# JiawangBian/SC-SfMLearner-Release

Measured on AMD Instinct MI355X. Metric: train images/sec (+ warp-loss ms/step) KITTI 256x832 RN18, higher is better.
Workload: dtype f32; 1 GPU; configs[1]: kitti 256x832, batch 12/GPU, 2 refs (seq 3), ResNet18 DispNet + ResNet18 PoseNet, ssim+mask+auto-mask, zeros padding, 1 scale; global_batch=12, parallelism=1 GPU, memory_format=contiguous (NCHW)

## Files before the change

### __graft_entry__.py

```python
import os
import sys

ROOT = os.path.dirname(os.path.abspath(__file__))
PKG = os.path.join(ROOT, "sc-sfmlearner-release_amd")
for p in (ROOT, PKG):
    if p not in sys.path:
        sys.path.insert(0, p)


REPORT_ORDER = ("dgrad", "vlog", "wrw", "decb", "enceval", "val", "dvis", "", "nets", "eval", "odom", "enc", "stem", "snip",
                "vis", "prep")


def build() -> None:
    from scsfm_hip import _lib, build as hip_build
    from scsfm_hip.libraries import ADDED, BEYOND, BY_NAME, FURTHER, LATER, NEWER, NEWEST, NEXT, REGISTRY
    libs = {row.name: _lib.CLib(hip_build.build_lib(row.name, force=False), row.header, row.abi, row.prefix)
            for row in REGISTRY}
    assert libs[""]._dll.scsfm_abi_version() == _lib.ABI_VERSION
    import inverse_warp
    import loss_functions
    import models
    from scsfm_hip import decoder, depth_eval, depth_vis, encoder, odometry, prepare, snippets, visualise
    from scsfm_hip import conv_wrw, decoder_bias, decoder_dgrad, encoder_eval, validation, validation_log
    from scsfm_hip import conv1x1, encoder_frozen, fusion, meshing, optim, raycast, tracking, training_state
    from scsfm_hip import confidence, rolling, similarity
    from oracle import scsfm_oracle
    for row in ADDED + FURTHER:
        print(f"[{row.tag}] {libs[row.name].path}: ABI {row.abi}, {len(libs[row.name].decls)} symbols of "
              f"include/{os.path.basename(row.header)}")
    for row in NEWER + NEWEST:
        print(f"[{row.tag}] {libs[row.name].path}: {len(libs[row.name].decls)} entry points resolved (ABI {row.abi})")
    for row in LATER:
        print(f"[{row.tag}] {libs[row.name].path}: {len(libs[row.name].decls)} entry points resolved")
    for row in NEXT:
        print(f"[{row.tag}] {libs[row.name].path}: {len(libs[row.name].decls)} entry points resolved (ABI {row.abi})")
    for name in REPORT_ORDER:
        print(f"[{BY_NAME[name].tag}] {libs[name].path}: {len(libs[name].decls)} entry points resolved")
        if name == "dgrad":
            for row in BEYOND:
                print(f"[{row.tag}] {libs[row.name].path}: {len(libs[row.name].decls)} entry points resolved (ABI "
                      f"{row.abi})")


def smoke() -> None:
    import torch

    import loss_functions as LF
    from oracle import scsfm_oracle as O
    from scsfm_hip import _lib, synth

    assert torch.cuda.is_available(), "smoke() needs a HIP device"
    lib = _lib.get()
    assert lib.path.endswith("libscsfm_hip.so")
    dev = torch.device("cuda:0")
    d = synth.make_batch(2, 128, 416, n_ref=2, seed=0, depth="smooth")

    def leaves(device):
        mv = lambda t: t.to(device).clone().requires_grad_(True)
        return ([mv(t) for t in d["tgt_depth"]], [[mv(t) for t in r] for r in d["ref_depths"]],
                [mv(p) for p in d["poses"]], [mv(p) for p in d["poses_inv"]])

    td, rd, ps, pi = leaves(dev)
    tgt, refs, K = d["tgt_img"].to(dev), [r.to(dev) for r in d["ref_imgs"]], d["intrinsics"].to(dev)
    photo, geom = LF.compute_photo_and_geometry_loss(tgt, refs, K, td, rd, ps, pi, 1, 1, 1, 1, "zeros")
    smooth = LF.compute_smooth_loss(td, tgt, rd, refs)
    (photo + 0.1 * smooth + 0.5 * geom).backward()
    torch.cuda.synchronize()

    td_c, rd_c, ps_c, pi_c = leaves("cpu")
    photo_c, geom_c = O.photo_and_geometry_loss(d["tgt_img"], d["ref_imgs"], d["intrinsics"], td_c, rd_c, ps_c, pi_c,
                                                1, 1, 1, 1, "zeros")
    smooth_c = O.smooth_loss(td_c, d["tgt_img"], rd_c, d["ref_imgs"])
    (photo_c + 0.1 * smooth_c + 0.5 * geom_c).backward()
    for name, a, b in (("photo", photo, photo_c), ("geom", geom, geom_c), ("smooth", smooth, smooth_c)):
        err = abs(float(a) - float(b))
        print(f"[smoke] {name}: hip {float(a):.7f} oracle {float(b):.7f} |d| {err:.2e}")
        assert err <= 1e-5, name
    pairs = [("g_tgt_depth", td[0].grad, td_c[0].grad), ("g_ref0_depth", rd[0][0].grad, rd_c[0][0].grad),
             ("g_ref1_depth", rd[1][0].grad, rd_c[1][0].grad), ("g_pose0", ps[0].grad, ps_c[0].grad),
             ("g_pose_inv1", pi[1].grad, pi_c[1].grad)]
    for name, a, b in pairs:
        scale = float(b.abs().max())
        bad = ((a.cpu() - b).abs() > 0.01 * scale).double().mean().item()
        print(f"[smoke] {name}: scale {scale:.3e} share of entries off by >1% of scale {bad:.2e}")
        assert bad <= 2e-3, name
    import torch.nn as nn
    from scsfm_hip import encoder as E
    assert _lib.get_stem().path.endswith("libscsfm_stem.so")
    xs = torch.randn(2, 4, 6, 8, device=dev)
    bn_a, bn_b = nn.BatchNorm2d(4).to(dev).train(), nn.BatchNorm2d(4).to(dev).train()
    f0, pooled = E.bn_act(xs, bn_a, pool=True)
    f0_ref = E.bn_act(xs, bn_b)
    assert torch.equal(f0, f0_ref) and torch.equal(pooled, E.max_pool(f0_ref))
    print("[smoke] stem: fused BatchNorm / ReLU / max-pool equals the separate ops")
    import numpy as np
    from scsfm_hip import visualise as V
    assert _lib.get_vis().path.endswith("libscsfm_vis.so")
    ramp = torch.linspace(0.05, 12.0, 70).reshape(2, 5, 7)
    for cmap, max_value in (("bone", None), ("rainbow", 10)):
        got = V.colourise(ramp.to(dev), colormap=cmap, max_value=max_value).cpu().numpy()
        table = V.colour_table(cmap)
        r = ramp.numpy()
        d = r.reshape(2, -1).max(axis=1)[:, None, None] if max_value is None else np.float32(max_value)
        xa = (r / d).astype(np.float32) * np.float32(len(table))
        want = table[np.clip(xa.astype(np.int64), 0, len(table) - 1)]
        assert got.shape == (2, 5, 7, 4) and np.array_equal(got, want), cmap
    print("[smoke] vis: bone and rainbow pictures of a ramp equal the table lookup")
    from scsfm_hip import depth_vis as DV
# ... 10 lines not shown
    print("[smoke] dvis: the magma picture of a depth ramp equals the table lookup")
    from scsfm_hip import validation as VA
    assert _lib.get_val().path.endswith("libscsfm_val.so")
    f32 = np.float32
    rng = np.random.default_rng(0)
    gt_v = rng.uniform(0.05, 90.0, (2, 20, 60)).astype(f32)
    disp_v = rng.uniform(0.01, 1.5, (2, 10, 30)).astype(f32)
    res = VA.depth_errors(torch.from_numpy(gt_v).to(dev), torch.from_numpy(disp_v).to(dev), "kitti", is_disp=True)
    got = VA.batch_mean(res)
    y1, y2, x1, x2 = int(0.40810811 * 20), int(0.99189189 * 20), int(0.03594771 * 60), int(0.96405229 * 60)
    want = np.zeros(6)
    for g, dsp in zip(gt_v, disp_v):
        p = (f32(1) / dsp)[np.arange(20) // 2][:, np.arange(60) // 2]
        ok = np.zeros((20, 60), bool)
        ok[y1:y2, x1:x2] = True
        ok &= (g > f32(0.1)) & (g < f32(80))
        g, p = g[ok], np.clip(p[ok], f32(1e-3), f32(80))
        p = p * np.sort(g)[(g.size - 1) // 2] / np.sort(p)[(p.size - 1) // 2]
        t = np.maximum(g / p, p / g)
        e = np.abs(g - p).astype(np.float64)
        want += [e.mean(), (e / g).mean(), (e * e / g).mean(), (t < 1.25).mean(), (t < 1.25 ** 2).mean(),
                 (t < 1.25 ** 3).mean()]
    want /= 2
    print(f"[smoke] val: abs_rel hip {got[1]:.7f} numpy {want[1]:.7f}; a1 hip {got[3]:.7f} numpy {want[3]:.7f}")
    assert res.count.cpu().numpy().min() > 100 and np.allclose(got, want, rtol=1e-6, atol=0), (got, want)
    table = VA.ValidationTable(4, dev)
    rows_v = [(0.25, 0.002, 1.5), (0.5, float("nan"), 0.75), (0.125, 0.004, 0.25)]
    for i, vals_v in zip((0, 1, 3), rows_v):
        table.add_losses(i, *torch.tensor(vals_v, device=dev))
    mean_v, n_v = table.finish()
    sums_v = [0.0] * 4
    for p_v, s_v, g_v in rows_v:
        sums_v = [a + float(f32(b)) for a, b in zip(sums_v, (p_v, p_v, s_v, g_v))]
    want_v = [s / 3 for s in sums_v] + [0.0] * 3
    print(f"[smoke] val: table of 3 present rows of 4: photo {mean_v[1]:.7f} host {want_v[1]:.7f}, smooth {mean_v[2]} "
          f"(a NaN row), geometry {mean_v[3]:.7f} host {want_v[3]:.7f}")
    assert n_v == 3 and np.isnan(mean_v[2]) and mean_v[:2] + mean_v[3:] == want_v[:2] + want_v[3:], (mean_v, want_v)
    import torch.nn.functional as F
    from scsfm_hip import encoder_eval as EE
    assert _lib.get_enceval().path.endswith("libscsfm_enceval.so")
    bn_e = nn.BatchNorm2d(4).to(dev)
    with torch.no_grad():
        bn_e.running_mean.copy_(torch.tensor([0.5, -1.0, 0.0, 2.0]))
        bn_e.running_var.copy_(torch.tensor([0.25, 1.0, 4.0, 0.5]))
        bn_e.weight.copy_(torch.tensor([1.0, -0.5, 2.0, 0.0]))
        bn_e.bias.copy_(torch.tensor([0.0, 0.1, -0.2, 0.3]))
    bn_e.eval()
    with torch.no_grad():
        f0_e, pooled_e = EE.bn_act(xs, bn_e, pool=True)
        want_e = F.relu(bn_e(xs))
        assert torch.equal(f0_e, EE.bn_act(xs, bn_e)) and torch.equal(pooled_e, F.max_pool2d(f0_e, 3, 2, 1))
        assert torch.equal(pooled_e, EE.max_pool(f0_e))
    err_e = float((f0_e - want_e).abs().max())
    print(f"[smoke] enceval: eval-mode BatchNorm / ReLU / max-pool, max |fused - ATen| {err_e:.2e}")
    assert err_e <= 1e-5
    from scsfm_hip import decoder_bias as DB
    assert _lib.get_decb().path.endswith("libscsfm_decb.so")
    conv_b = nn.Conv2d(4, 3, 3).to(dev)
    xb = torch.randn(2, 4, 9, 11, device=dev)
    want_b = F.pad(F.elu(conv_b(xb)), (1, 1, 1, 1), mode="reflect")
    want_h = 10 * torch.sigmoid(conv_b(xb)) + 0.01
    (want_b.sum() + want_h.sum()).backward()
    want_gb = conv_b.bias.grad.clone()
    conv_b.bias.grad = None
    raw = F.conv2d(xb, conv_b.weight, None)
    got_b, got_h = DB.elu_pad(raw, conv_b.bias), DB.disp_head(raw, conv_b.bias, 10, 0.01)
    (got_b.sum() + got_h.sum()).backward()
    err_b = float((conv_b.bias.grad - want_gb).abs().max() / want_gb.abs().max())
    print(f"[smoke] decb: bias folded into elu_pad and disp_head, relative bias-gradient difference {err_b:.2e}")
    assert torch.equal(got_b, want_b) and float((got_h - want_h).abs().max()) <= 1e-6 and err_b <= 1e-5
    _smoke_wrw(dev)
    _smoke_vlog(dev)
    _smoke_dgrad(dev)
    _smoke_fbn(dev)
    _smoke_opt(dev)
    _smoke_pw(dev)
    _smoke_fuse(dev)
    _smoke_mesh(dev)
    _smoke_cast(dev)
    _smoke_track(dev)
    _smoke_conf(dev)
    _smoke_roll(dev)
    _smoke_sim3(dev)
    print("[smoke] ok")


def _smoke_cast(dev) -> None:
    import numpy as np
    import torch

    from scsfm_hip import _lib
    from scsfm_hip import fusion as FU
    assert _lib.get_cast().path.endswith("libscsfm_cast.so")
    nx, ny, nz = 12, 10, 9
    z, y, x = np.meshgrid(np.arange(nz), np.arange(ny), np.arange(nx), indexing="ij")
    t = ((np.sqrt((x - 5.3) ** 2 + (y - 4.6) ** 2 + (z - 4.1) ** 2) - 3.2) / 3).clip(-1, 1).astype(np.float32)
    vol = FU.Volume((nx, ny, nz), (-0.6, -0.5, 0.3), 0.1, device=dev)
    vol.planes[0].copy_(torch.from_numpy(t))
    vol.planes[1].fill_(1.0)
    vol.planes[2:].fill_(0.5)
    centre = np.array([-0.6 + 0.1 * 5.8, -0.5 + 0.1 * 5.1, 0.3 + 0.1 * 4.6])
    c2w = np.concatenate([np.eye(3), [[centre[0]], [centre[1]], [-0.3]]], axis=1)[None]
    K = torch.tensor([[20.0, 0, 8.0], [0, 20.0, 6.0], [0, 0, 1]], device=dev)
    args = (torch.from_numpy(c2w).to(dev), K, (12, 16), 0.0, 1.5)
    got, plain = vol.raycast(*args), vol.raycast(*args, cull=False)
    for a, b in zip(got, plain):
        assert torch.equal(a.view(torch.uint8), b.view(torch.uint8))
    hits = int((got.depth > 0).sum())
    d = float(got.depth[0, 6, 8])
    want = centre[2] + 0.3 - 0.32
    assert hits > 40 and abs(d - want) < 0.025, (hits, d, want)
    assert float(got.normal[0, 2, 6, 8]) < -0.99 and int(got.shade[0, 6, 8]) >= 250 and got.rgb[0, 6, 8].tolist() == [128] * 3
    print(f"[smoke] cast: a sphere in a 12 x 10 x 9 volume from a 12 x 16 camera: {hits} pixels with a hit, the same bits "
          f"with and without the brick cull; the central depth {d:.4f} against {want:.4f}")


def _smoke_conf(dev) -> None:
    import numpy as np
    import torch

    from scsfm_hip import _lib, confidence
    from scsfm_hip import fusion as FU
    assert _lib.get_conf().path.endswith("libscsfm_conf.so")
    K = torch.tensor([[16.0, 0, 7.5], [0, 16.0, 5.5], [0, 0, 1]], device=dev)
    c2w = np.stack([np.concatenate([np.eye(3), [[0.125 * k], [0.0], [0.0]]], axis=1) for k in range(3)])
    c2w = torch.from_numpy(c2w).to(dev)
    depth = torch.full((3, 12, 16), 2.0, device=dev)
    flat = confidence.weights(depth, c2w, K, radius=1, is_disp=False, max_depth=4.0)
    met = int((flat == 1).sum())
    assert bool(((flat == 0) | (flat == 1)).all()) and met > 3 * 10 * 13, met
    depth[1, 4:8, 6:10] = 1.5
    w = confidence.weights(depth, c2w, K, radius=1, is_disp=False, max_depth=4.0)
    low = float(w[1, 4:8, 6:10].max())
    assert low < 0.9 and torch.equal(w[1, 9:11], flat[1, 9:11]), low
    vols = []
    for weight in (None, torch.ones_like(w), w):
        vol = FU.Volume((24, 16, 12), (-1.0, -0.8, 1.6), 0.1, device=dev)
        vol.integrate(depth, None, c2w, K, is_disp=False, max_depth=4.0, weight=weight)
        vols.append(vol.planes)
    assert torch.equal(vols[0].view(torch.int32), vols[1].view(torch.int32)) and not torch.equal(vols[0], vols[2])
    assert float(vols[2][1].max()) <= 3.0 and float(vols[2][1].max()) > 1.0
    print(f"[smoke] conf: three flat 12 x 16 frames a pixel apart: {met} weights of exactly 1, the rest 0; a nearer patch "
          f"weighs at most {low:.4f}; a weight of ones fuses to the unweighted bits")


def _smoke_roll(dev) -> None:
    import numpy as np
    import torch

    from scsfm_hip import _lib, rolling
    assert _lib.get_roll().path.endswith("libscsfm_roll.so")
    K = torch.tensor([[16.0, 0, 7.5], [0, 16.0, 5.5], [0, 0, 1]], device=dev)
    c2w = np.stack([np.concatenate([np.eye(3), [[0.125 * k], [0.0], [0.0]]], axis=1) for k in range(3)])
    c2w = torch.from_numpy(c2w).to(dev)
    yy = torch.arange(12, device=dev, dtype=torch.float32)[None, :, None]
    depth = (1.0 + 0.05 * yy).expand(3, 12, 16).contiguous()
    vol = rolling.RollingVolume((24, 16, 20), (-1.0, -0.75, 0.5), 0.0625, device=dev)
    assert vol.nbytes == 40 * 24 * 16 * 20 and vol.offset == (0, 0, 0) and vol.origin == vol.origin0
    vol.integrate(depth, None, c2w, K, is_disp=False, max_depth=4.0)
    before = vol.planes.clone()
    full = vol.extract(1.0)[0]
    out = vol.shift((8, 0, 10), 1.0)[0]
    want = torch.zeros_like(before)
    want[:, :10, :, :16] = before[:, 10:, :, 8:]
    assert torch.equal(vol.planes.view(torch.int32), want.view(torch.int32))
    assert vol.offset == (8, 0, 10) and vol.origin == (-0.5, -0.75, 1.125)
# ... 91 lines not shown
    w[:, :, 10:] = 0
    vol = FU.Volume((nx, ny, nz), (-0.6, -0.5, 0.3), 0.1, device=dev)
    vol.planes[0].copy_(torch.from_numpy(t))
    vol.planes[1].copy_(torch.from_numpy(w))
    vol.planes[2:].fill_(0.5)
    seen, neg = w >= 1, t < 0
    corner = lambda a, k: a[(k >> 2):nz - 1 + (k >> 2), ((k >> 1) & 1):ny - 1 + ((k >> 1) & 1), (k & 1):nx - 1 + (k & 1)]
    n_vert, is_axial = 0, []
    edge = np.zeros((nz, ny, nx, 7), bool)
    for e, k in enumerate((1, 2, 4, 3, 5, 6, 7)):
        dz, dy, dx = k >> 2, (k >> 1) & 1, k & 1
        a = (slice(0, nz - dz), slice(0, ny - dy), slice(0, nx - dx))
        b = (slice(dz, nz), slice(dy, ny), slice(dx, nx))
        edge[a + (e,)] = seen[a] & seen[b] & (neg[a] != neg[b])
    n_vert = int(edge.sum())
    is_axial = (np.flatnonzero(edge.reshape(-1)) % 7) < 3
    n_tri = 0
    for tet in ((0, 1, 3, 7), (0, 1, 5, 7), (0, 2, 3, 7), (0, 2, 6, 7), (0, 4, 5, 7), (0, 4, 6, 7)):
        ok = np.logical_and.reduce([corner(seen, k) for k in tet])
        inside = sum(corner(neg, k).astype(int) for k in tet)
        n_tri += int((ok & ((inside == 1) | (inside == 3))).sum() + 2 * (ok & (inside == 2)).sum())
    xyz, rgb, tri = vol.extract_mesh(1.0)
    pts, cols = vol.extract(1.0)
    assert xyz.shape == (n_vert, 3) and rgb.shape == (n_vert, 3) and tri.shape == (n_tri, 3) and n_tri > 100
    assert tri.dtype == torch.int32 and int(tri.min()) >= 0 and int(tri.max()) < n_vert
    keep = torch.from_numpy(is_axial).to(dev)
    assert torch.equal(xyz[keep].view(torch.int32), pts.view(torch.int32)) and torch.equal(rgb[keep], cols)
    print(f"[smoke] mesh: a cut sphere in a 12 x 10 x 9 volume: {n_vert} vertices and {n_tri} triangles as numpy counts "
          f"them; the {len(pts)} vertices on the grid's edges equal the surface points bit for bit")


def _smoke_fuse(dev) -> None:
    import numpy as np
    import torch

    from scsfm_hip import _lib
    from scsfm_hip import fusion as FU
    assert _lib.get_fuse().path.endswith("libscsfm_fuse.so")
    f32 = np.float32
    rng = np.random.default_rng(11)
    H, W, dims, origin, voxel, trunc, max_depth = 6, 8, (12, 10, 9), (-0.6, -0.5, 0.3), f32(0.1), f32(0.3), f32(3.0)
    K = np.array([[6, 0, 3.5], [0, 6, 2.5], [0, 0, 1]], f32)
    c2w = np.array([[[1, 0, 0, x], [0, 1, 0, 0.05], [0, 0, 1, 0]] for x in (-0.25, 0.5)], np.float64)
    disp = (1 / (0.8 + 0.02 * rng.random((2, 1, H, W)))).astype(f32)
    disp[0, 0, 1, 2], disp[1, 0, 4, 5] = 0.01, np.nan
    img = rng.standard_normal((2, 3, H, W)).astype(f32)
    vol = FU.Volume(dims, origin, float(voxel), float(trunc), max_weight=64.0, device=dev, frames_per_launch=2)
    vol.integrate(*(torch.from_numpy(a).to(dev) for a in (disp, img, c2w, K)), is_disp=True, near=0.05,
                  max_depth=float(max_depth))
    axis = lambda o, n: f32(o) + (np.arange(n, dtype=f32) + f32(0.5)) * voxel
    x, y, z = axis(origin[0], 12)[None, None, :], axis(origin[1], 10)[None, :, None], axis(origin[2], 9)[:, None, None]
    planes = np.zeros((5, 9, 10, 12), f32)
    t, w = planes[0], planes[1]
    with np.errstate(all="ignore"):
        for f in range(2):
            tr = (-c2w[f, :, 3]).astype(f32)
            qx, qy, qz = ((x + f32(0) * y) + f32(0) * z) + tr[0], ((f32(0) * x + y) + f32(0) * z) + tr[1], \
                ((f32(0) * x + f32(0) * y) + z) + tr[2]
            a, b = ((K[0, 0] * qx) / qz + K[0, 2]) + f32(0.5), ((K[1, 1] * qy) / qz + K[1, 2]) + f32(0.5)
            ok = (qz > f32(0.05)) & (a >= 0) & (a < f32(W)) & (b >= 0) & (b < f32(H))
            px, py = np.where(ok, a, 0).astype(np.int32), np.where(ok, b, 0).astype(np.int32)
            d = f32(1) / disp[f, 0][py, px]
            sdf = d - qz
            ok &= (d > 0) & (d <= max_depth) & ~(sdf < -trunc)
            w1 = w + f32(1)
            t[...] = np.where(ok, (t * w + np.minimum(f32(1), sdf / trunc)) / w1, t)
            for ch in range(3):
                col = img[f, ch][py, px] * f32(0.225) + f32(0.45)
                planes[2 + ch] = np.where(ok, (planes[2 + ch] * w + col) / w1, planes[2 + ch])
            w[...] = np.where(ok, np.minimum(w1, f32(64)), w)
    assert planes.dtype == f32 and w.max() == 2 and torch.equal(vol.planes.cpu(), torch.from_numpy(planes))
    seen, neg = w >= 1, t < 0
    n_z = int((seen[:-1] & seen[1:] & (neg[:-1] != neg[1:])).sum())
    n_y = int((seen[:, :-1] & seen[:, 1:] & (neg[:, :-1] != neg[:, 1:])).sum())
    n_x = int((seen[:, :, :-1] & seen[:, :, 1:] & (neg[:, :, :-1] != neg[:, :, 1:])).sum())
    xyz, rgb = vol.extract(min_weight=1)
    assert xyz.shape == (n_x + n_y + n_z, 3) and rgb.shape == xyz.shape and n_z > 20
    zs = xyz[:, 2].cpu().numpy()
    print(f"[smoke] fuse: two frames into a 12 x 10 x 9 volume equal the numpy restatement bit for bit; {len(zs)} surface "
          f"points, depth {zs.min():.3f} .. {zs.max():.3f} of a surface at 0.80 .. 0.82")
    assert 0.75 < zs.min() and zs.max() < 0.87


def _smoke_pw(dev) -> None:
    import torch
    import torch.nn.functional as F

    from scsfm_hip import _lib
    from scsfm_hip import conv1x1 as PW
    assert _lib.get_pw().path.endswith("libscsfm_pw.so")
    g = torch.Generator().manual_seed(9)
    xp = torch.randn(2, 64, 7, 11, generator=g).to(dev).requires_grad_(True)
    wp = (torch.randn(128, 64, 1, 1, generator=g) / 8).to(dev).requires_grad_(True)
    gy = torch.randn(2, 128, 4, 6, generator=g).to(dev)
    old = torch.backends.cudnn.deterministic, torch.backends.cudnn.benchmark
    torch.backends.cudnn.deterministic, torch.backends.cudnn.benchmark = True, False
    try:
        y, y_ref = PW.conv1x1(xp, wp, None, 2), F.conv2d(xp, wp, None, 2)
    finally:
        torch.backends.cudnn.deterministic, torch.backends.cudnn.benchmark = old
    assert torch.equal(y, y_ref)
    gx_w, gw_w = PW.data_grad(gy, wp.detach(), 7, 11), PW.weight_grad(xp.detach(), gy, 2)
    gx_m, gw_m = torch.autograd.grad(y_ref, (xp, wp), gy)
    x64, w64 = (t.detach().double().requires_grad_(True) for t in (xp, wp))
    gx_64, gw_64 = torch.autograd.grad(F.conv2d(x64, w64, None, 2), (x64, w64), gy.double())
    xa, wa = (t.detach().double().abs().requires_grad_(True) for t in (xp, wp))
    sx_64, sw_64 = torch.autograd.grad(F.conv2d(xa, wa, None, 2), (xa, wa), gy.double().abs())
    u8 = 8 * 2.0 ** -24
    for name, got, miopen, want, s in (("weight", gw_w, gw_m, gw_64, sw_64), ("data", gx_w, gx_m, gx_64, sx_64)):
        err, err_m = (got - want).abs(), float((miopen - want).abs().max())
        print(f"[smoke] pw: {name} gradient of a 64 -> 128 stride-2 1x1 convolution, max |hip - fp64| "
              f"{float(err.max()):.2e} (MIOpen's {err_m:.2e})")
        assert bool((err <= 2 * err_m + u8 * s).all()), name
    assert bool((gx_w[:, :, 1::2, :] == 0).all()) and bool((gx_w[:, :, :, 1::2] == 0).all())
    if (64, 128, 2) in PW.ROUTED and (64, 128, 2) in PW.ROUTED_DGRAD:
        gx_f, gw_f = torch.autograd.grad(y, (xp, wp), gy)
        assert torch.equal(gx_f, gx_w) and torch.equal(gw_f, gw_w)


def _smoke_opt(dev) -> None:
    import numpy as np
    import torch

    from scsfm_hip import _lib
    from scsfm_hip import optim as OP
    assert _lib.get_opt().path.endswith("libscsfm_opt.so")
    f32 = np.float32
    g = torch.Generator().manual_seed(7)
    shapes, lrs, wd, betas, eps = ((7,), (4, 6), (2 * OP.CHUNK + 3,), (3, 5, 5)), (1e-3, 1e-2), 0.01, (0.9, 0.999), 1e-8
    host = [torch.randn(s, generator=g) for s in shapes]
    params = [torch.nn.Parameter(t.to(dev)) for t in host]
    opt = OP.Adam([{"params": params[:2], "lr": lrs[0]}, {"params": params[2:], "lr": lrs[1]}], betas=betas, eps=eps,
                  weight_decay=wd)
    p = [t.numpy().copy() for t in host]
    m, v = [np.zeros_like(a) for a in p], [np.zeros_like(a) for a in p]
    b1c, b2, b2c, e, w = f32(1.0 - betas[0]), f32(betas[1]), f32(1.0 - betas[1]), f32(eps), f32(wd)
    for step in (1, 2, 3):
        grads = [torch.randn(s, generator=g) for s in shapes]
        for q, gr in zip(params, grads):
            q.grad = gr.to(dev)
        opt.step()
        for k, gr in enumerate(grads):
            step_size = f32(lrs[k // 2] / (1 - betas[0] ** step))
            bc2_sqrt = f32((1 - betas[1] ** step) ** 0.5)
            gk = gr.numpy() + w * p[k]
            m[k] = m[k] + b1c * (gk - m[k])
            v[k] = v[k] * b2 + (b2c * gk) * gk
            p[k] = p[k] - step_size * (m[k] / (np.sqrt(v[k]) / bc2_sqrt + e))
    state = opt.state_dict()["state"]
    for k in range(4):
        assert p[k].dtype == f32 and torch.equal(params[k].detach().cpu(), torch.from_numpy(p[k])), k
        assert torch.equal(state[k]["exp_avg"].cpu(), torch.from_numpy(m[k])), k
        assert torch.equal(state[k]["exp_avg_sq"].cpu(), torch.from_numpy(v[k])), k
        assert float(state[k]["step"]) == 3.0
    print("[smoke] opt: three Adam steps of four tensors in one launch each equal the numpy restatement bit for bit")


def _smoke_fbn(dev) -> None:
    import torch
    import torch.nn as nn
    import torch.nn.functional as F

    from scsfm_hip import _lib
    from scsfm_hip import encoder_frozen as EF
    assert _lib.get_fbn().path.endswith("libscsfm_fbn.so")
    g = torch.Generator().manual_seed(5)
# ... 106 lines not shown
```

### sc-sfmlearner-release_amd/models/resnet_encoder.py

```python
from __future__ import absolute_import, division, print_function

import numpy as np
import torch
import torch.nn as nn


_encoder_ops = None


def _E():
    global _encoder_ops
    if _encoder_ops is None:
        from scsfm_hip import encoder
        _encoder_ops = encoder
    return _encoder_ops


_encoder_eval_ops = None


def _EV():
    global _encoder_eval_ops
    if _encoder_eval_ops is None:
        from scsfm_hip import encoder_eval
        _encoder_eval_ops = encoder_eval
    return _encoder_eval_ops


_encoder_frozen_ops = None


def _EF():
    global _encoder_frozen_ops
    if _encoder_frozen_ops is None:
        from scsfm_hip import encoder_frozen
        _encoder_frozen_ops = encoder_frozen
    return _encoder_frozen_ops


def _fused_applies(x, *bns):
    return x.is_cuda and _E().applies(x, *bns)


def _eval_applies(x, *bns):
    return x.is_cuda and _EV().applies(x, *bns)


def _frozen_applies(x, *bns, relu=True):
    return x.is_cuda and not any(bn.training for bn in bns) and _EF().applies(x, *bns, relu=relu)


def _bn_act(x, bn, act, identity=None):
    if _fused_applies(x, bn) and (identity is None or _fused_applies(identity)):
        return _E().bn_act(x, bn, identity, relu=act is not None)
    if _frozen_applies(x, bn, relu=act is not None) and (identity is None or _frozen_applies(identity)):
        return _EF().bn_act(x, bn, identity, relu=act is not None)
    if _eval_applies(x, bn) and (identity is None or _eval_applies(identity)):
        return _EV().bn_act(x, bn, identity, relu=act is not None)
    out = bn(x)
    if identity is not None:
        out = out + identity
    return out if act is None else act(out)


_conv1x1_ops = None


def _PW():
    global _conv1x1_ops
    if _conv1x1_ops is None:
        from scsfm_hip import conv1x1
        _conv1x1_ops = conv1x1
    return _conv1x1_ops


def _downsample(ds, x):
    conv, bn = ds[0], ds[1]
    hip = x.is_cuda and (bn.training or (_EF().is_frozen(bn) and _EF().enabled()))
    y = _PW().conv(conv, x) if hip else conv(x)
    return _bn_act(y, bn, None)


def _conv3x3(cin, cout, stride=1):
    return nn.Conv2d(cin, cout, kernel_size=3, stride=stride, padding=1, bias=False)


class BasicBlock(nn.Module):
    expansion = 1

    def __init__(self, inplanes, planes, stride=1, downsample=None):
        super().__init__()
        self.conv1 = _conv3x3(inplanes, planes, stride)
        self.bn1 = nn.BatchNorm2d(planes)
        self.relu = nn.ReLU(inplace=True)
        self.conv2 = _conv3x3(planes, planes)
        self.bn2 = nn.BatchNorm2d(planes)
        self.downsample = downsample

    def forward(self, x):
        identity = x if self.downsample is None else _downsample(self.downsample, x)
        out = _bn_act(self.conv1(x), self.bn1, self.relu)
        return _bn_act(self.conv2(out), self.bn2, self.relu, identity)

    def forward_reference(self, x):
        identity = x if self.downsample is None else self.downsample(x)
        out = self.relu(self.bn1(self.conv1(x)))
        out = self.bn2(self.conv2(out))
        return self.relu(out + identity)


class Bottleneck(nn.Module):
    expansion = 4

    def __init__(self, inplanes, planes, stride=1, downsample=None):
        super().__init__()
        self.conv1 = nn.Conv2d(inplanes, planes, kernel_size=1, bias=False)
        self.bn1 = nn.BatchNorm2d(planes)
        self.conv2 = _conv3x3(planes, planes, stride)
        self.bn2 = nn.BatchNorm2d(planes)
        self.conv3 = nn.Conv2d(planes, planes * 4, kernel_size=1, bias=False)
        self.bn3 = nn.BatchNorm2d(planes * 4)
        self.relu = nn.ReLU(inplace=True)
        self.downsample = downsample

    def forward(self, x):
        identity = x if self.downsample is None else _downsample(self.downsample, x)
        out = _bn_act(self.conv1(x), self.bn1, self.relu)
        out = _bn_act(self.conv2(out), self.bn2, self.relu)
        return _bn_act(self.conv3(out), self.bn3, self.relu, identity)

    def forward_reference(self, x):
        identity = x if self.downsample is None else self.downsample(x)
        out = self.relu(self.bn1(self.conv1(x)))
        out = self.relu(self.bn2(self.conv2(out)))
        out = self.bn3(self.conv3(out))
        return self.relu(out + identity)


class ResNet(nn.Module):

    def __init__(self, block, layers, num_classes=1000, num_input_images=1):
        super().__init__()
        self.inplanes = 64
        self.conv1 = nn.Conv2d(num_input_images * 3, 64, kernel_size=7, stride=2, padding=3, bias=False)
        self.bn1 = nn.BatchNorm2d(64)
        self.relu = nn.ReLU(inplace=True)
        self.maxpool = nn.MaxPool2d(kernel_size=3, stride=2, padding=1)
        self.layer1 = self._make_layer(block, 64, layers[0])
        self.layer2 = self._make_layer(block, 128, layers[1], stride=2)
        self.layer3 = self._make_layer(block, 256, layers[2], stride=2)
        self.layer4 = self._make_layer(block, 512, layers[3], stride=2)
        self.avgpool = nn.AdaptiveAvgPool2d((1, 1))
        self.fc = nn.Linear(512 * block.expansion, num_classes)
        for m in self.modules():
            if isinstance(m, nn.Conv2d):
                nn.init.kaiming_normal_(m.weight, mode='fan_out', nonlinearity='relu')
            elif isinstance(m, nn.BatchNorm2d):
                nn.init.constant_(m.weight, 1)
                nn.init.constant_(m.bias, 0)

    def _make_layer(self, block, planes, blocks, stride=1):
        downsample = None
        if stride != 1 or self.inplanes != planes * block.expansion:
            downsample = nn.Sequential(
                nn.Conv2d(self.inplanes, planes * block.expansion, kernel_size=1, stride=stride, bias=False),
                nn.BatchNorm2d(planes * block.expansion))
        layers = [block(self.inplanes, planes, stride, downsample)]
        self.inplanes = planes * block.expansion
        layers += [block(self.inplanes, planes) for _ in range(1, blocks)]
        return nn.Sequential(*layers)


_CFG = {18: (BasicBlock, [2, 2, 2, 2]), 50: (Bottleneck, [3, 4, 6, 3])}


def imagenet_weights_path(num_layers):
    import os
    root = os.environ.get("SCSFM_IMAGENET_WEIGHTS")
    if not root:
        return None
    path = os.path.join(root, "resnet{}.pth".format(num_layers))
    return path if os.path.exists(path) else None


class ResnetEncoder(nn.Module):

    def __init__(self, num_layers, pretrained, num_input_images=1):
        super().__init__()
        if num_layers not in _CFG:
            raise ValueError("{} is not a valid number of resnet layers".format(num_layers))
        block, layers = _CFG[num_layers]
        self.num_ch_enc = np.array([64, 64, 128, 256, 512])
        if num_layers > 34:
            self.num_ch_enc[1:] *= 4
        self.encoder = ResNet(block, layers, num_input_images=num_input_images)
        if pretrained:
            path = imagenet_weights_path(num_layers)
            if path is None:
                raise RuntimeError("ImageNet-pretrained weights are not reachable offline: set SCSFM_IMAGENET_WEIGHTS "
                                   "to a directory holding resnet{}.pth, or use --with-pretrain 0".format(num_layers))
            loaded = torch.load(path, map_location="cpu")
            loaded['conv1.weight'] = torch.cat([loaded['conv1.weight']] * num_input_images, 1) / num_input_images
            self.encoder.load_state_dict(loaded)
        for p in self.encoder.fc.parameters():
            p.requires_grad_(False)

    def forward(self, input_image):
        e = self.encoder
        x = e.conv1(input_image)
        if _fused_applies(x, e.bn1) and _E().pool_applies(x):
            f0, pooled = _E().bn_act(x, e.bn1, relu=True, pool=True)
# ... 30 lines not shown
```

### sc-sfmlearner-release_amd/scsfm_hip/config.py

```python
from __future__ import annotations

_hint = (1.0, 0.5)
_hint_dev = {}


def set_weight_hint(w_photo, w_geom):
    global _hint
    if w_photo is None:
        _hint = None
        return
    import numpy as np
    _hint = (float(np.float32(w_photo)), float(np.float32(w_geom)))
    for t in _hint_dev.values():
        t.copy_(t.new_tensor(_hint))


def weight_hint():
    return _hint


def hint_tensor(device):
    if _hint is None:
        return None
    import torch
# ... 24 lines not shown
def set_smooth_rides_along(on):
    global _smooth_rides
    _smooth_rides = bool(on)


_errors_torch = None


def errors_on_torch():
    global _errors_torch
    if _errors_torch is None:
        import os
        _errors_torch = os.environ.get("SCSFM_ERRORS_TORCH", "0") == "1"
    return _errors_torch


def set_errors_on_torch(on):
    global _errors_torch
    _errors_torch = bool(on)


_decoder_bias = None


def decoder_bias_folded():
    global _decoder_bias
    if _decoder_bias is None:
        import os
        _decoder_bias = os.environ.get("SCSFM_DECODER_BIAS", "1") != "0"
    return _decoder_bias


def set_decoder_bias_folded(on):
    global _decoder_bias
    _decoder_bias = None if on is None else bool(on)


_decoder_wrw = None


def decoder_wrw():
    global _decoder_wrw
    if _decoder_wrw is None:
        import os
        _decoder_wrw = os.environ.get("SCSFM_DECODER_WRW", "1") != "0"
    return _decoder_wrw


def set_decoder_wrw(on):
    global _decoder_wrw
    _decoder_wrw = None if on is None else bool(on)


_decoder_dgrad = None


def decoder_dgrad():
    global _decoder_dgrad
    if _decoder_dgrad is None:
        import os
        _decoder_dgrad = os.environ.get("SCSFM_DECODER_DGRAD", "1") != "0"
    return _decoder_dgrad


def set_decoder_dgrad(on):
    global _decoder_dgrad
    _decoder_dgrad = None if on is None else bool(on)


_conv1x1_bwd = None


def conv1x1_bwd():
    global _conv1x1_bwd
    if _conv1x1_bwd is None:
        import os
        _conv1x1_bwd = os.environ.get("SCSFM_CONV1X1_BWD", "1") != "0"
    return _conv1x1_bwd


def set_conv1x1_bwd(on):
    global _conv1x1_bwd
    _conv1x1_bwd = None if on is None else bool(on)
```

### sc-sfmlearner-release_amd/scsfm_hip/libraries.py

```python
from __future__ import annotations

import os
from typing import NamedTuple

HERE = os.path.dirname(os.path.abspath(__file__))
INCLUDE = os.path.join(os.path.dirname(os.path.dirname(HERE)), "include")


class Library(NamedTuple):
    name: str
    abi: int
    tag: str
    what: str

    @property
    def csrc(self):
        return os.path.join(os.path.dirname(HERE), "csrc_" + self.name if self.name else "csrc")

    @property
    def header(self):
        return os.path.join(INCLUDE, f"scsfm_{self.name or 'hip'}.h")

    @property
    def lib(self):
        return os.path.join(HERE, f"libscsfm_{self.name or 'hip'}.so")

    @property
    def prefix(self):
        return f"scsfm_{self.name}_" if self.name else "scsfm_"


TABLE = (
    Library("", 9, "build", "the loss path"),
    Library("nets", 1, "build", "the depth decoder's fused glue"),
    Library("eval", 1, "build", "depth evaluation with median scaling"),
    Library("odom", 1, "build", "the pose chain of test_vo.py and KITTI odometry evaluation"),
    Library("enc", 1, "build", "the ResNet encoder's fused BatchNorm / ReLU / residual / max-pool glue"),
    Library("stem", 1, "build", "the ResNet stem's BatchNorm / ReLU fused with its max-pool"),
    Library("snip", 1, "build", "the 5-frame snippet pose evaluation of test_pose.py"),
    Library("prep", 1, "build:prep", "the resize and the Velodyne depth maps of data/prepare_train_data.py"),
    Library("vis", 1, "build:vis", "the input normalisation, the per-image maximum and the colour-mapped pictures of "
                                   "run_inference.py"),
    Library("dvis", 1, "build:dvis", "the scaled prediction, the colour range and the magma pictures of eval_depth.py "
                                     "--vis_dir"),
    Library("val", 2, "val:build", "the validation pass of train.py: the ground-truth metrics of --with-gt and the "
                                   "per-batch table of --shard-validation"),
    Library("enceval", 1, "enceval:build", "the ResNet encoder's eval-mode BatchNorm / ReLU / residual / max-pool glue"),
    Library("decb", 1, "decb:build", "the depth decoder's glue with the convolutions' biases folded in"),
    Library("wrw", 1, "wrw:build", "the weight gradient of the depth decoder's low-channel 3x3 convolutions"),
    Library("vlog", 1, "vlog:build", "the validation pictures of train.py --log-output"),
    Library("dgrad", 1, "dgrad:build", "the backward of the depth decoder's full-resolution tail"),
)
LATER = (
    Library("fbn", 1, "fbn:build", "the backward of the ResNet encoder's BatchNorm with frozen statistics (train.py "
                                   "--freeze-bn)"),
)
BY_NAME = {row.name: row for row in TABLE + LATER}
NEWER = (
    Library("opt", 1, "opt:build", "Adam over every parameter tensor in one launch (train.py --optimizer hip)"),
)
ROWS = TABLE + LATER + NEWER
NEWEST = (
    Library("pw", 1, "pw:build", "the weight and stride-2 data gradients of the encoders' 1x1 down-sample convolutions"),
)
EVERY = ROWS + NEWEST
NEXT = (
    Library("fuse", 1, "fuse:build", "the TSDF fusion of predicted depth and poses and the surface points of "
                                     "reconstruct.py"),
)
ALL = EVERY + NEXT
BEYOND = (
    Library("mesh", 1, "mesh:build", "the triangle mesh of a fused volume's surface by marching tetrahedra (reconstruct.py "
                                     "--mesh)"),
)
LIBRARIES = ALL + BEYOND
FURTHER = (
    Library("cast", 1, "cast:build", "the ray cast of a fused volume from camera poses: depth, normals, colour and shaded "
                                     "pictures (reconstruct.py --render)"),
)
CATALOGUE = LIBRARIES + FURTHER
ADDED = (
    Library("track", 1, "track:build", "the frame-to-model tracking of predicted depth against the ray-cast model by "
                                       "point-to-plane ICP (reconstruct.py --refine-poses)"),
    Library("conf", 1, "conf:build", "the depth consistency of a frame with its neighbours as a per-pixel confidence and "
                                     "the TSDF fusion weighed by it (reconstruct.py --consistency-weight)"),
    Library("roll", 1, "roll:build", "the shift of a volume that follows the camera by whole voxels and the surface points "
                                     "that leave with it (reconstruct.py --follow)"),
    Library("sim3", 1, "sim3:build", "the frame-to-model tracking of predicted depth with a scale of its own per frame: "
                                     "point-to-plane ICP over seven degrees of freedom, the scale solved only where it is "
                                     "observable (reconstruct.py --refine-scale)"),
)
REGISTRY = CATALOGUE + ADDED
_FIND = {row.name: row for row in REGISTRY}


def find(name):
    return _FIND[name]


SUMMARY = "\n".join(f"    {os.path.basename(row.lib):22s} {os.path.basename(row.csrc) + '/':14s} "
                    f"include/{os.path.basename(row.header):16s} {row.what}" for row in LIBRARIES)
SINCE = "\n".join(f"    {os.path.basename(row.lib):22s} {os.path.basename(row.csrc) + '/':14s} "
                  f"include/{os.path.basename(row.header):16s} {row.what}" for row in FURTHER + ADDED)
```

Measured before the change: 153.4 images/s.

## Add HIP MFMA weight-gradient kernel for ResNet encoder 3x3 convolutions

Adds a custom HIP kernel that computes the weight gradient of the encoders' 3x3 stride-1/2 convolutions using fp32 MFMA instructions. Each block writes a partial into a workspace, and an fp64 summation kernel reduces the partials. The BasicBlock and Bottleneck forwards are routed through a custom autograd function that keeps MIOpen for the forward pass and the data gradient but replaces the weight gradient for selected channel/stride shapes. The aim is to beat MIOpen's backward-weights path, at the cost of an extra workspace allocation and a second reduction launch per convolution.

```diff
diff --git a/__graft_entry__.py b/__graft_entry__.py
--- a/__graft_entry__.py
+++ b/__graft_entry__.py
@@ -24,7 +24,7 @@
     from scsfm_hip import decoder, depth_eval, depth_vis, encoder, odometry, prepare, snippets, visualise
     from scsfm_hip import conv_wrw, decoder_bias, decoder_dgrad, encoder_eval, validation, validation_log
     from scsfm_hip import conv1x1, encoder_frozen, fusion, meshing, optim, raycast, tracking, training_state
-    from scsfm_hip import confidence, rolling, similarity
+    from scsfm_hip import confidence, conv3x3, rolling, similarity
     from oracle import scsfm_oracle
     for row in ADDED + FURTHER:
         print(f"[{row.tag}] {libs[row.name].path}: ABI {row.abi}, {len(libs[row.name].decls)} symbols of "
@@ -201,6 +201,7 @@
     _smoke_conf(dev)
     _smoke_roll(dev)
     _smoke_sim3(dev)
+    _smoke_ewrw(dev)
     print("[smoke] ok")
 
 
@@ -458,6 +459,37 @@
     assert 0.75 < zs.min() and zs.max() < 0.87
 
 
+def _smoke_ewrw(dev) -> None:
+    import torch
+    import torch.nn.functional as F
+
+    from scsfm_hip import _lib
+    from scsfm_hip import conv3x3 as C3
+    assert _lib.get_ewrw().path.endswith("libscsfm_ewrw.so")
+    g = torch.Generator().manual_seed(11)
+    xp = torch.randn(2, 64, 7, 11, generator=g).to(dev).requires_grad_(True)
+    wp = (torch.randn(128, 64, 3, 3, generator=g) / 24).to(dev).requires_grad_(True)
+    gy = torch.randn(2, 128, 4, 6, generator=g).to(dev)
+    old = torch.backends.cudnn.deterministic, torch.backends.cudnn.benchmark
+    torch.backends.cudnn.deterministic, torch.backends.cudnn.benchmark = True, False
+    try:
+        y, y_ref = C3.conv3x3(xp, wp, 2), F.conv2d(xp, wp, None, 2, 1)
+        assert torch.equal(y, y_ref)
+        gx, gw = torch.autograd.grad(y, (xp, wp), gy)
+        gx_m, gw_m = torch.autograd.grad(y_ref, (xp, wp), gy)
+    finally:
+        torch.backends.cudnn.deterministic, torch.backends.cudnn.benchmark = old
+    xc, gc = xp.detach().cpu(), gy.cpu()
+    gw_64 = torch.nn.grad.conv2d_weight(xc.double(), wp.shape, gc.double(), stride=2, padding=1)
+    gw_32 = torch.nn.grad.conv2d_weight(xc, wp.shape, gc, stride=2, padding=1)
+    err, err_m = float((gw.cpu() - gw_64).abs().max()), float((gw_m.cpu() - gw_64).abs().max())
+    err_c = float((gw_32 - gw_64).abs().max())
+    print(f"[smoke] ewrw: weight gradient of a 64 -> 128 stride-2 3x3 convolution, max |hip - fp64| {err:.2e} "
+          f"(MIOpen's {err_m:.2e}, the CPU's fp32 {err_c:.2e})")
+    assert err <= 3 * err_c and torch.equal(gx, gx_m)
+    assert torch.equal(gw, C3.weight_grad(xp.detach(), gy, 2))
+
+
 def _smoke_pw(dev) -> None:
     import torch
     import torch.nn.functional as F
diff --git a/include/scsfm_ewrw.h b/include/scsfm_ewrw.h
--- /dev/null
+++ b/include/scsfm_ewrw.h
@@ -0,0 +1,26 @@
+#ifndef SCSFM_EWRW_H_
+#define SCSFM_EWRW_H_
+
+#include <stddef.h>
+
+#ifndef SCSFM_ERR_ARG
+#define SCSFM_ERR_ARG (-1)
+#endif
+
+#ifdef __cplusplus
+extern "C" {
+#endif
+
+int scsfm_ewrw_abi_version(void);
+int scsfm_ewrw_source_id(char* buf, size_t n);
+int scsfm_ewrw_covers(int Cin, int Cout, int stride);
+size_t scsfm_ewrw_ws_bytes(int B, int Cin, int Cout, int H, int W, int stride);
+int scsfm_ewrw_partials(int B, int Cin, int Cout, int H, int W, int stride);
+int scsfm_ewrw_conv3x3_f32(int B, int Cin, int Cout, int H, int W, int stride, const float* x, const float* dy, float* dw,
+                           void* ws, size_t ws_bytes, void* stream);
+
+#ifdef __cplusplus
+}
+#endif
+
+#endif
diff --git a/sc-sfmlearner-release_amd/csrc_ewrw/scsfm_enc_wrw.hip b/sc-sfmlearner-release_amd/csrc_ewrw/scsfm_enc_wrw.hip
--- /dev/null
+++ b/sc-sfmlearner-release_amd/csrc_ewrw/scsfm_enc_wrw.hip
@@ -0,0 +1,309 @@
+#include <hip/hip_runtime.h>
+
+#include "scsfm_ewrw.h"
+
+#ifndef SCSFM_WRW_F32X4
+typedef float f32x4 __attribute__((ext_vector_type(4)));
+#endif
+
+namespace scsfm_ewrw {
+
+constexpr int kWave = 64;
+constexpr int kHalf = 256;
+constexpr int kThreads = 2 * kHalf;
+constexpr int kKP = 32;
+constexpr int kSP = kKP + 2;
+constexpr int kSlots = 256;
+constexpr int kRed = 16 * 16 * 9;
+constexpr int kSlices = 8, kPerBlock = 256 / kSlices;
+
+__host__ __device__ inline int imin(int a, int b) { return a < b ? a : b; }
+__host__ __device__ inline int imax(int a, int b) { return a > b ? a : b; }
+__host__ __device__ inline int ceil_div(int a, int b) { return (a + b - 1) / b; }
+
+template <int S, int CW>
+struct Geo {
+  static constexpr int RH = kKP / CW;
+  static constexpr int PR = S * (RH - 1) + 3, PC = S * (CW - 1) + 3;
+  static constexpr int PE = PR * PC;
+  static constexpr int PL = PE + (6 - PE % 4) % 4;
+  static constexpr int WM = S == 1 ? 2 : 4, WN = S == 1 ? 2 : 1;
+  static constexpr int TM = 32 * WM, TN = 32 * WN;
+  static constexpr int HALF = TM * kSP + TN * PL;
+  static constexpr int ND = TM / 8;
+  static constexpr int PP = kHalf / PE;
+  static constexpr int NX = (TN + PP - 1) / PP;
+  static_assert(PP >= 1, "a halo fits the threads of a half");
+  static_assert(2 * HALF >= 4 * kRed, "the epilogue's exchange fits the staging area");
+};
+constexpr int tile_m(int s) { return s == 1 ? 64 : 128; }
+constexpr int tile_n(int s) { return s == 1 ? 64 : 32; }
+
+template <int S, int CW>
+static __global__ __launch_bounds__(kThreads) void wrw_kernel(int Cin, int Cout, int H, int W, int Ho, int Wo, int segs,
+                                                              int chunks_img, int nchunks, int tiles_n,
+                                                              const float* __restrict__ x, const float* __restrict__ dy,
+                                                              float* __restrict__ ws) {
+  using G = Geo<S, CW>;
+  __shared__ float smem[2 * G::HALF];
+
+  const int tid = threadIdx.x, half = tid >> 8, t8 = tid & (kHalf - 1);
+  const int lane = tid & (kWave - 1), wave = (tid >> 6) & 3;
+  const int wm = wave / G::WN, wn = wave % G::WN;
+  const int l15 = lane & 15, quad = lane >> 4;
+  const int q32 = t8 & 31, r8 = t8 >> 5;
+  const int P = gridDim.x, g = blockIdx.x;
+  const int co0 = (blockIdx.y / tiles_n) * G::TM, ci0 = (blockIdx.y % tiles_n) * G::TN;
+  float* const ds = smem + half * G::HALF;
+  float* const xs = ds + G::TM * kSP;
+
+  f32x4 acc[2][2][9];
+#pragma unroll
+  for (int m = 0; m < 2; ++m)
+#pragma unroll
+    for (int c = 0; c < 2; ++c)
+#pragma unroll
+      for (int tap = 0; tap < 9; ++tap) acc[m][c][tap] = f32x4{0.f, 0.f, 0.f, 0.f};
+
+  float pd[G::ND], px[G::NX];
+  bool p_in = false, p_ok = false;
+  const int py_l = q32 / CW, px_l = q32 % CW;
+  const int pl_l = t8 / G::PE, rm_l = t8 - pl_l * G::PE;
+  const int row_l = rm_l / G::PC, col_l = rm_l - row_l * G::PC;
+  const bool act_l = pl_l < G::PP;
+  float* const xl = xs + pl_l * G::PL + row_l * G::PC +
+                    (S == 1 ? col_l : ((col_l & 1) ? CW + 1 + (col_l >> 1) : (col_l >> 1)));
+  auto prefetch = [&](int t) {
+    const int c = 2 * t + half;
+    const bool valid = c < nchunks;
+    const int n = c / chunks_img, rem = c - n * chunks_img;
+    const int band = rem / segs, seg = rem - band * segs;
+    const int h0 = band * G::RH, w0 = seg * CW;
+    const int hh = h0 + py_l, ww = w0 + px_l;
+    const bool in = valid && hh < Ho && ww < Wo;
+    const unsigned dg = 4u * (unsigned)((((n * Cout + co0 + r8) * Ho + hh) * Wo) + ww);
+    const unsigned plane = 4u * 8u * (unsigned)(Ho * Wo);
+#pragma unroll
+    for (int j = 0; j < G::ND; ++j)
+      pd[j] = *(const float*)((const char*)dy + (in ? dg + j * plane : 0u));
+    p_in = in;
+    const int y = S * h0 - 1 + row_l, xx = S * w0 - 1 + col_l;
+    const bool ok = valid && act_l && y >= 0 && y < H && xx >= 0 && xx < W;
+    const unsigned xg = 4u * (unsigned)((((n * Cin + ci0 + pl_l) * H + y) * W) + xx);
+    const unsigned step = 4u * (unsigned)(G::PP * H * W);
+#pragma unroll
+    for (int j = 0; j < G::NX; ++j)
+      px[j] = *(const float*)((const char*)x + ((ok && pl_l + G::PP * j < G::TN) ? xg + j * step : 0u));
+    p_ok = ok;
+  };
+  auto commit = [&]() {
+#pragma unroll
+    for (int j = 0; j < G::ND; ++j) ds[(r8 + 8 * j) * kSP + q32] = p_in ? pd[j] : 0.f;
+#pragma unroll
+    for (int j = 0; j < G::NX; ++j)
+      if (act_l && pl_l + G::PP * j < G::TN) xl[j * G::PP * G::PL] = p_ok ? px[j] : 0.f;
+  };
+
+  const float* __restrict__ ap = ds + (wm * 32 + l15) * kSP + quad;
+  const float* __restrict__ bp = xs + (wn * 32 + l15) * G::PL + quad;
+  const int npairs = (nchunks + 1) / 2;
+  if (g < npairs) prefetch(g);
+  for (int t = g; t < npairs; t += P) {
+    __syncthreads();
+    commit();
+    __syncthreads();
+    if (t + P < npairs) prefetch(t + P);
+#pragma unroll
+    for (int k = 0; k < kKP / 4; ++k) {
+      const int py = (4 * k) / CW, px0 = (4 * k) % CW;
+      float a[2], b[2][9];
+#pragma unroll
+      for (int m = 0; m < 2; ++m) a[m] = ap[m * 16 * kSP + 4 * k];
+#pragma unroll
+      for (int c = 0; c < 2; ++c)
+#pragma unroll
+        for (int r = 0; r < 3; ++r)
+#pragma unroll
+          for (int s = 0; s < 3; ++s) {
+            const int off = S == 1 ? s : (s == 0 ? 0 : (s == 1 ? CW + 1 : 1));
+            b[c][r * 3 + s] = bp[c * 16 * G::PL + (S * py + r) * G::PC + px0 + off];
+          }
+#pragma unroll
+      for (int m = 0; m < 2; ++m)
+#pragma unroll
+        for (int c = 0; c < 2; ++c)
+#pragma unroll
+          for (int tap = 0; tap < 9; ++tap)
+            acc[m][c][tap] = __builtin_amdgcn_mfma_f32_16x16x4f32(a[m], b[c][tap], acc[m][c][tap], 0, 0, 0);
+#ifndef __HOSTSIM__
+      __builtin_amdgcn_sched_barrier(0);
+#endif
+    }
+  }
+
+  float* const red = smem + wave * kRed;
+  float* __restrict__ out = ws + (size_t)g * ((size_t)Cout * Cin * 9);
+#pragma unroll
+  for (int m = 0; m < 2; ++m)
+#pragma unroll
+    for (int c = 0; c < 2; ++c) {
+      __syncthreads();
+      if (half == 1) {
+#pragma unroll
+        for (int tap = 0; tap < 9; ++tap)
+#pragma unroll
+          for (int i = 0; i < 4; ++i) red[((quad * 4 + i) * 16 + l15) * 9 + tap] = acc[m][c][tap][i];
+      }
+      __syncthreads();
+      if (half == 0) {
+#pragma unroll
+        for (int tap = 0; tap < 9; ++tap)
+#pragma unroll
+          for (int i = 0; i < 4; ++i) red[((quad * 4 + i) * 16 + l15) * 9 + tap] += acc[m][c][tap][i];
+      }
+      __syncthreads();
+      float* __restrict__ o = out + ((size_t)(co0 + wm * 32 + m * 16) * Cin + ci0 + wn * 32 + c * 16) * 9;
+#pragma unroll
+      for (int rr = 0; rr < 8; ++rr) {
+        const int row = half * 8 + rr;
+        for (int e = lane; e < 144; e += kWave) o[(size_t)row * Cin * 9 + e] = red[row * 144 + e];
+      }
+    }
+}
+
+static __global__ __launch_bounds__(256) void sum_kernel(int G, int E, const float* __restrict__ ws,
+                                                         float* __restrict__ dw) {
+  __shared__ double part[kSlices][kPerBlock];
+  const int j = threadIdx.x & (kPerBlock - 1), sl = threadIdx.x / kPerBlock;
+  const int e = blockIdx.x * kPerBlock + j;
+  double s = 0.0;
+  if (e < E) {
+#pragma unroll 8
+    for (int g = sl; g < G; g += kSlices) s += (double)ws[(size_t)g * E + e];
+  }
+  part[sl][j] = s;
+  __syncthreads();
+  if (sl == 0 && e < E) {
+    double t = part[0][j];
+#pragma unroll
+    for (int p = 1; p < kSlices; ++p) t += part[p][j];
+    dw[e] = (float)t;
+  }
+}
+
+static __global__ __launch_bounds__(256) void sum_few_kernel(int G, int E, const float* __restrict__ ws,
+                                                             float* __restrict__ dw) {
+  const int e = blockIdx.x * 256 + threadIdx.x;
+  if (e >= E) return;
+  double t = 0.0;
+  for (int g = 0; g < G; ++g) t += (double)ws[(size_t)g * E + e];
+  dw[e] = (float)t;
+}
+
+inline bool channels(int c) { return c == 64 || c == 128 || c == 256 || c == 512; }
+inline bool covers(int Cin, int Cout, int stride) {
+  return channels(Cin) && channels(Cout) && (stride == 1 || (stride == 2 && Cout >= 128));
+}
+
+struct Plan {
+  int Ho, Wo, cw, segs, chunks_img, nchunks, tiles_n, tiles, P, E;
+};
+
+inline bool plan_of(int B, int Cin, int Cout, int H, int W, int stride, Plan& p) {
+  if (B <= 0 || H <= 0 || W <= 0 || !covers(Cin, Cout, stride)) return false;
+  const long long lim = 1ll << 29;
+  p.Ho = (H - 1) / stride + 1;
+  p.Wo = (W - 1) / stride + 1;
+  if ((long long)B * Cin * H * W >= lim || (long long)B * Cout * p.Ho * p.Wo >= lim) return false;
+  long long best = -1;
+  p.cw = 0;
+  for (int cw = 32; cw >= 4; cw /= 2) {
+    const int rh = kKP / cw;
+    const long long padded = (long long)ceil_div(p.Wo, cw) * cw * ((long long)ceil_div(p.Ho, rh) * rh);
+    if (best < 0 || padded < best) best = padded, p.cw = cw;
+  }
+  if ((long long)B * best + 2 * kKP >= lim) return false;
+  if ((long long)stride * (p.Ho + 8) >= lim || (long long)stride * (p.Wo + 32) >= lim) return false;
+  p.segs = ceil_div(p.Wo, p.cw);
+  p.chunks_img = p.segs * ceil_div(p.Ho, kKP / p.cw);
+  p.nchunks = B * p.chunks_img;
+  p.tiles_n = Cin / tile_n(stride);
+  p.tiles = (Cout / tile_m(stride)) * p.tiles_n;
+  p.P = imin((p.nchunks + 1) / 2, imax(1, kSlots / p.tiles));
+  p.E = Cout * Cin * 9;
+  return true;
+}
+
+inline int launch_status() { return (int)hipGetLastError(); }
+
+template <int S>
+inline void launch(const Plan& p, int Cin, int Cout, int H, int W, const float* x, const float* dy, float* ws,
+                   hipStream_t st) {
+  const dim3 grid(p.P, p.tiles), block(kThreads);
+#define SCSFM_EWRW_LAUNCH(CW)                                                                                         \
+  hipLaunchKernelGGL((wrw_kernel<S, CW>), grid, block, 0, st, Cin, Cout, H, W, p.Ho, p.Wo, p.segs, p.chunks_img,      \
+                     p.nchunks, p.tiles_n, x, dy, ws)
+  switch (p.cw) {
+    case 32: SCSFM_EWRW_LAUNCH(32); break;
+    case 16: SCSFM_EWRW_LAUNCH(16); break;
+    case 8: SCSFM_EWRW_LAUNCH(8); break;
+    default: SCSFM_EWRW_LAUNCH(4); break;
+  }
+#undef SCSFM_EWRW_LAUNCH
+}
+
+}
+
+using namespace scsfm_ewrw;
+
+extern "C" {
+
+int scsfm_ewrw_abi_version(void) { return 1; }
+
+#ifndef SCSFM_SOURCE_ID
+#define SCSFM_SOURCE_ID "unknown"
+#endif
+static const char g_source_tag[] __attribute__((used)) = "scsfm-source-id:" SCSFM_SOURCE_ID;
+int scsfm_ewrw_source_id(char* buf, size_t n) {
+  const volatile char* id = g_source_tag + 16;
+  if (!buf || n == 0) return -1;
+  size_t i = 0;
+  for (; i + 1 < n && id[i]; ++i) buf[i] = id[i];
+  buf[i] = 0;
+  return 0;
+}
+
+int scsfm_ewrw_covers(int Cin, int Cout, int stride) { return covers(Cin, Cout, stride) ? 1 : 0; }
+
+size_t scsfm_ewrw_ws_bytes(int B, int Cin, int Cout, int H, int W, int stride) {
+  Plan p;
+  if (!plan_of(B, Cin, Cout, H, W, stride, p)) return 0;
+  return sizeof(float) * (size_t)p.P * p.E;
+}
+
+int scsfm_ewrw_partials(int B, int Cin, int Cout, int H, int W, int stride) {
+  Plan p;
+  return plan_of(B, Cin, Cout, H, W, stride, p) ? p.P : 0;
+}
+
+int scsfm_ewrw_conv3x3_f32(int B, int Cin, int Cout, int H, int W, int stride, const float* x, const float* dy, float* dw,
+                           void* ws, size_t ws_bytes, void* stream) {
+  Plan p;
+  if (!plan_of(B, Cin, Cout, H, W, stride, p) || !x || !dy || !dw || !ws || ((size_t)ws & 3) ||
+      ws_bytes < sizeof(float) * (size_t)p.P * p.E)
+    return SCSFM_ERR_ARG;
+  (void)hipGetLastError();
+  hipStream_t st = (hipStream_t)stream;
+  if (stride == 1)
+    launch<1>(p, Cin, Cout, H, W, x, dy, (float*)ws, st);
+  else
+    launch<2>(p, Cin, Cout, H, W, x, dy, (float*)ws, st);
+  if (const int rc = launch_status()) return rc;
+  if (p.P <= kSlices)
+    hipLaunchKernelGGL(sum_few_kernel, dim3(ceil_div(p.E, 256)), dim3(256), 0, st, p.P, p.E, (const float*)ws, dw);
+  else
+    hipLaunchKernelGGL(sum_kernel, dim3(ceil_div(p.E, kPerBlock)), dim3(256), 0, st, p.P, p.E, (const float*)ws, dw);
+  return launch_status();
+}
+
+}
diff --git a/sc-sfmlearner-release_amd/models/resnet_encoder.py b/sc-sfmlearner-release_amd/models/resnet_encoder.py
--- a/sc-sfmlearner-release_amd/models/resnet_encoder.py
+++ b/sc-sfmlearner-release_amd/models/resnet_encoder.py
@@ -85,6 +85,19 @@
     return nn.Conv2d(cin, cout, kernel_size=3, stride=stride, padding=1, bias=False)
 
 
+_conv3x3_ops = None
+
+
+def _c3(conv, bn, x):
+    global _conv3x3_ops
+    if not (x.is_cuda and (bn.training or (_EF().is_frozen(bn) and _EF().enabled()))):
+        return conv(x)
+    if _conv3x3_ops is None:
+        from scsfm_hip import conv3x3
+        _conv3x3_ops = conv3x3
+    return _conv3x3_ops.conv(conv, x)
+
+
 class BasicBlock(nn.Module):
     expansion = 1
 
@@ -99,8 +112,8 @@
 
     def forward(self, x):
         identity = x if self.downsample is None else _downsample(self.downsample, x)
-        out = _bn_act(self.conv1(x), self.bn1, self.relu)
-        return _bn_act(self.conv2(out), self.bn2, self.relu, identity)
+        out = _bn_act(_c3(self.conv1, self.bn1, x), self.bn1, self.relu)
+        return _bn_act(_c3(self.conv2, self.bn2, out), self.bn2, self.relu, identity)
 
     def forward_reference(self, x):
         identity = x if self.downsample is None else self.downsample(x)
@@ -126,7 +139,7 @@
     def forward(self, x):
         identity = x if self.downsample is None else _downsample(self.downsample, x)
         out = _bn_act(self.conv1(x), self.bn1, self.relu)
-        out = _bn_act(self.conv2(out), self.bn2, self.relu)
+        out = _bn_act(_c3(self.conv2, self.bn2, out), self.bn2, self.relu)
         return _bn_act(self.conv3(out), self.bn3, self.relu, identity)
 
     def forward_reference(self, x):
diff --git a/sc-sfmlearner-release_amd/scsfm_hip/config.py b/sc-sfmlearner-release_amd/scsfm_hip/config.py
--- a/sc-sfmlearner-release_amd/scsfm_hip/config.py
+++ b/sc-sfmlearner-release_amd/scsfm_hip/config.py
@@ -130,3 +130,19 @@
 def set_conv1x1_bwd(on):
     global _conv1x1_bwd
     _conv1x1_bwd = None if on is None else bool(on)
+
+
+_encoder_wrw = None
+
+
+def encoder_wrw():
+    global _encoder_wrw
+    if _encoder_wrw is None:
+        import os
+        _encoder_wrw = os.environ.get("SCSFM_ENCODER_WRW", "1") != "0"
+    return _encoder_wrw
+
+
+def set_encoder_wrw(on):
+    global _encoder_wrw
+    _encoder_wrw = None if on is None else bool(on)
diff --git a/sc-sfmlearner-release_amd/scsfm_hip/conv3x3.py b/sc-sfmlearner-release_amd/scsfm_hip/conv3x3.py
--- /dev/null
+++ b/sc-sfmlearner-release_amd/scsfm_hip/conv3x3.py
@@ -0,0 +1,92 @@
+from __future__ import annotations
+
+import torch
+import torch.nn.functional as F
+
+from . import _lib, config
+from .capi import _stream
+
+CHANNELS = (64, 128, 256, 512)
+STRIDES = (1, 2)
+ROUTED = {(64, 64, 1), (64, 128, 2), (128, 128, 1), (128, 256, 2), (256, 256, 1)}
+
+
+def covers(cin, cout, stride):
+    return (int(cin) in CHANNELS and int(cout) in CHANNELS and int(stride) in STRIDES
+            and (int(stride) == 1 or int(cout) >= 128))
+
+
+def _triple(m):
+    return int(m.weight.shape[1]), int(m.weight.shape[0]), int(m.stride[0])
+
+
+def _plain3x3(x, m):
+    w = m.weight
+    return (x.is_cuda and x.dtype == torch.float32 and x.dim() == 4 and x.is_contiguous() and x.numel() > 0
+            and w.is_cuda and w.dtype == torch.float32 and w.is_contiguous() and tuple(w.shape[2:]) == (3, 3)
+            and m.bias is None and tuple(m.stride) in ((1, 1), (2, 2)) and tuple(m.padding) == (1, 1)
+            and tuple(m.dilation) == (1, 1) and m.groups == 1 and m.padding_mode == "zeros"
+            and x.shape[1] == w.shape[1])
+
+
+def applies(x, m):
+    return bool(config.encoder_wrw() and torch.is_grad_enabled() and _plain3x3(x, m) and _triple(m) in ROUTED)
+
+
+def _out_size(n, stride):
+    return (n - 1) // stride + 1
+
+
+def weight_grad(x, gy, stride):
+    B, Cin, H, W = x.shape
+    Cout = gy.shape[1]
+    if not (x.is_cuda and gy.is_cuda and x.dtype == gy.dtype == torch.float32 and x.is_contiguous()
+            and gy.is_contiguous() and tuple(gy.shape) == (B, Cout, _out_size(H, stride), _out_size(W, stride))):
+        raise ValueError(f"scsfm_hip.conv3x3: CUDA fp32 contiguous x[B, Cin, H, W] and gy[B, Cout, Ho, Wo] only "
+                         f"(got {x.device} {x.dtype} {tuple(x.shape)} and {gy.device} {gy.dtype} {tuple(gy.shape)})")
+    lib = _lib.get_ewrw()
+    n = lib.size("scsfm_ewrw_ws_bytes", B, Cin, Cout, H, W, stride)
+    if n == 0:
+        raise ValueError(f"scsfm_hip.conv3x3: no kernel for {Cin} -> {Cout} channels, stride {stride}, at {B} x {H} x {W}")
+    ws = torch.empty(n // 4, dtype=torch.float32, device=x.device)
+    dw = torch.empty((Cout, Cin, 3, 3), dtype=torch.float32, device=x.device)
+    lib.call("scsfm_ewrw_conv3x3_f32", B, Cin, Cout, H, W, stride, x.data_ptr(), gy.data_ptr(), dw.data_ptr(),
+             ws.data_ptr(), n, _stream(x))
+    return dw
+
+
+class _Conv3x3(torch.autograd.Function):
+    @staticmethod
+    def forward(ctx, x, weight, stride):
+        ctx.save_for_backward(x, weight)
+        ctx.stride = stride
+        return F.conv2d(x, weight, None, stride, 1)
+
+    @staticmethod
+    def backward(ctx, gy):
+        x, weight = ctx.saved_tensors
+        s = ctx.stride
+        gy = gy.contiguous()
+        triple = (int(weight.shape[1]), int(weight.shape[0]), s)
+        gx = gw = None
+
+        def aten(k):
+            mask = [k == 0, k == 1, False]
+            return torch.ops.aten.convolution_backward(gy, x, weight, None, [s, s], [1, 1], [1, 1], False, [0, 0], 1,
+                                                       mask)[k]
+
+        if ctx.needs_input_grad[0]:
+            gx = aten(0)
+        if ctx.needs_input_grad[1]:
+            gw = weight_grad(x, gy, s) if triple in ROUTED else aten(1)
+        return gx, gw, None
+
+
+def conv3x3(x, weight, stride=1):
+    return _Conv3x3.apply(x, weight, int(stride))
+
+
+def conv(m, x):
+    if applies(x, m):
+        return conv3x3(x, m.weight, int(m.stride[0]))
+    return m(x)
diff --git a/sc-sfmlearner-release_amd/scsfm_hip/libraries.py b/sc-sfmlearner-release_amd/scsfm_hip/libraries.py
--- a/sc-sfmlearner-release_amd/scsfm_hip/libraries.py
+++ b/sc-sfmlearner-release_amd/scsfm_hip/libraries.py
@@ -89,6 +89,8 @@
     Library("sim3", 1, "sim3:build", "the frame-to-model tracking of predicted depth with a scale of its own per frame: "
                                      "point-to-plane ICP over seven degrees of freedom, the scale solved only where it is "
                                      "observable (reconstruct.py --refine-scale)"),
+    Library("ewrw", 1, "ewrw:build", "the weight gradient of the ResNet encoders' 3x3 convolutions, stride 1 and 2, read "
+                                     "as NCHW lies"),
 )
 REGISTRY = CATALOGUE + ADDED
 _FIND = {row.name: row for row in REGISTRY}
```

New measurement: 154.4 images/s (median of 4 runs). About the same (+0.6%).
